# edwindn/rl-agent-for-qubit-array-tuning

Measured on NVIDIA B200. Metric: ground_state_pixels_per_s, higher is better.
Workload: dtype f64

## Files before the change

### rl-agent-for-qubit-array-tuning_b200/csrc/qd_api.cu

```cuda
#include <cuda_runtime.h>
#include <stdarg.h>
#include <stdio.h>
#include <string.h>

#include <new>
#include <stdlib.h>

#include <algorithm>
#include <chrono>
#include <type_traits>
#include <vector>

#include "qd_kernels.cuh"
#include "qd_tunnel.cuh"
#include "qd_tunnel_noda.cuh"
#include "qd_tunnel_enum.cuh"
#include "qd_normalise.cuh"

static_assert(sizeof(qd_scan) == 480, "qd_scan must be 480 bytes (multiple of 16 for the TMA bulk copy)");
static_assert(sizeof(qd_scan) % 16 == 0, "qd_scan size");

struct qd_ctx {
  int device = 0;
  int sm_count = 0;
// ... 155 lines not shown
int issue(qd_ctx* ctx, void (*fn)(P...), long long grid, int threads, size_t smem, cudaStream_t stream, const A&... args) {
  if (smem) {
    const int rc = configure_kernel(ctx, (const void*)fn, smem);
    if (rc) return rc;
  }
  fn<<<(unsigned)std::min(grid, 0x7fffffffLL), threads, smem, stream>>>(args...);
  QD_CUDA(ctx, cudaGetLastError());
  ctx->launches += 1;
  return QD_OK;
}

int order_after_last_launch(qd_ctx* ctx, cudaStream_t stream) {
  if (ctx->have_last && ctx->last_stream != stream) QD_CUDA(ctx, cudaStreamWaitEvent(stream, ctx->last_launch, 0));
  return QD_OK;
}
int mark_launch(qd_ctx* ctx, cudaStream_t stream) {
  QD_CUDA(ctx, cudaEventRecord(ctx->last_launch, stream));
  ctx->last_stream = stream;
  ctx->have_last = true;
  return QD_OK;
}

struct PixelItems { int warps; long long grid; };
PixelItems plan_pixel_items(const qd_ctx* ctx, qd::KArgs& a, long long max_pix, int warps_per_sm) {
  const long long want_items = (long long)ctx->sm_count * warps_per_sm * 4;
  const long long ppi = std::min<long long>(std::max<long long>(((long long)a.n_scan * max_pix) / want_items, 1), 64);
  a.rows_per_item = (int)ppi;
  a.items_per_scan = (int)((max_pix + ppi - 1) / ppi);
  const long long items = (long long)a.n_scan * a.items_per_scan;
  const int warps = (items < (long long)ctx->sm_count * 4) ? 1 : 4;
  return {warps, (items + warps - 1) / warps};
}

int primary_then_fixup(qd_ctx* ctx, const qd::KArgs& g, const PixelItems& p, kernel_fn primary, const qd::KArgs& pa,
                       kernel_fn fallback, int fallback_slot_bytes, bool fix, cudaStream_t stream) {
  if (primary) {
    const int rc = issue(ctx, primary, p.grid, p.warps * 32, (size_t)pa.slot_bytes * p.warps, stream, pa);
    if (rc) return rc;
  }
  if (!fix) return QD_OK;
  qd::KArgs fa = g;
  fa.slot_bytes = fallback_slot_bytes;
  long long grid = p.grid;
  if (primary) {
    fa.fixup = 1;
    fa.mark_ppi = g.rows_per_item;
    fa.rows_per_item = (g.rows_per_item % 8 == 0) ? 8 : g.rows_per_item;
    fa.items_per_scan = (int)((ctx->up_max_pix + fa.rows_per_item - 1) / fa.rows_per_item);
    grid = ((long long)fa.n_scan * fa.items_per_scan + p.warps - 1) / p.warps;
    grid = std::min<long long>(grid, (long long)ctx->sm_count * 32);
  }
  return issue(ctx, fallback, grid, p.warps * 32, (size_t)fa.slot_bytes * p.warps, stream, fa);
}

int tunnel_ground_state(qd_ctx* ctx, int n_scan, const qd_scan* d_scans, const double* d_points, unsigned flags,
                        cudaStream_t stream) {
  const int N = ctx->L.n_dot;
  const kernel_fn gs = pick_dots<2>(N, [](auto n) { return qd::qd_tunnel_gs_kernel<decltype(n)::value>; });
  if (!gs) return fail(ctx, QD_ERR_UNSUPPORTED, "tunnel path needs 2..8 dots, got %d", N);
  int rc = grow(ctx, &ctx->d_nbar, &ctx->nbar_cap, (size_t)ctx->up_pixels * N * sizeof(double));
  if (rc) return rc;
  qd::KArgs g;
  memset(&g, 0, sizeof(g));
  g.L = ctx->L; g.records = ctx->d_records; g.scans = d_scans; g.points = d_points; g.z_out = nullptr;
  g.n_out = nullptr; g.nbar = ctx->d_nbar; g.n_scan = n_scan; g.n_type = QD_N_NONE; g.flags = flags;
  g.status = ctx->d_status;
  g.topt = 7;
  if (const char* e = getenv("QDSIM_TUNNEL_OPT")) g.topt = atoi(e) & 7;
  const long long max_pix = ctx->up_max_pix;
  const char* mono_e = getenv("QDSIM_TUNNEL_MONO");
  if (mono_e && mono_e[0] == '1') {
    g.slot_bytes = qd::qd_tunnel_slot_bytes(ctx->L);
    const PixelItems p = plan_pixel_items(ctx, g, max_pix, 12);
    return issue(ctx, gs, p.grid, p.warps * 32, (size_t)g.slot_bytes * p.warps, stream, g);
  }
  const kernel_fn kr = pick_dots<2>(N, [](auto n) { return qd::qd_tunnel_relax_kernel<decltype(n)::value>; });
  const kernel_fn ks = pick_dots<2>(N, [](auto n) { return qd::qd_tunnel_select_kernel<decltype(n)::value>; });
  const kernel_fn ke = pick_dots<2>(N, [](auto n) { return qd::qd_tunnel_eigen_kernel<decltype(n)::value>; });
  const char* sel_e = getenv("QDSIM_SELECT");
  const kernel_fn ks2 = (sel_e && sel_e[0] == 'b')
                            ? nullptr
                            : pick_dots<4>(N, [](auto n) { return qd::qd_tunnel_select2_kernel<decltype(n)::value>; });
  const char* eig_e = getenv("QDSIM_EIGEN");
  const bool no_fixup = eig_e && eig_e[0] == 'n';
  const kernel_fn ke2 = (eig_e && eig_e[0] == 'h')
                            ? nullptr
                            : pick_dots<2>(N, [](auto n) { return qd::qd_tunnel_eigen2_kernel<decltype(n)::value>; });
  long long chunk_pix = 8LL << 20;
  if (const char* e = getenv("QDSIM_TUNNEL_CHUNK_PIX")) chunk_pix = atoll(e) > 0 ? atoll(e) : chunk_pix;
  const long long spc = std::min<long long>(std::max<long long>(chunk_pix / max_pix, 1), n_scan);
  rc = grow(ctx, &ctx->d_tfloor, &ctx->tfloor_cap, (size_t)spc * max_pix * 8);
  if (rc) return rc;
  rc = grow(ctx, &ctx->d_tkeys, &ctx->tkeys_cap, (size_t)spc * max_pix * 256);
  if (rc) return rc;
  rc = grow(ctx, &ctx->d_tpot, &ctx->tpot_cap, (size_t)spc * max_pix * 128);
  if (rc) return rc;
  g.tfloor = ctx->d_tfloor;
  g.tpot = ctx->d_tpot;
  g.tkeys = ctx->d_tkeys;
  g.tstride = max_pix;
  for (long long c0 = 0; c0 < n_scan; c0 += spc) {
    g.scans = d_scans + c0;
    g.n_scan = (int)std::min<long long>(spc, n_scan - c0);
    qd::KArgs r = g;
    r.rows_per_item = (int)std::min<long long>(1024, max_pix);
    r.items_per_scan = (int)((max_pix + r.rows_per_item - 1) / r.rows_per_item);
    rc = issue(ctx, kr, (long long)r.n_scan * r.items_per_scan, 128, qd::qd_tunnel_relax_smem_bytes(ctx->L), stream, r);
    if (rc) return rc;
    const PixelItems p = plan_pixel_items(ctx, g, max_pix, 16);
    qd::KArgs sa = g;
    sa.slot_bytes = qd::qd_tunnel_select2_slot_bytes(ctx->L);
    rc = primary_then_fixup(ctx, g, p, ks2, sa, ks, qd::qd_tunnel_select_slot_bytes(ctx->L), true, stream);
    if (rc) return rc;
    qd::KArgs ea = g;
    ea.e2_kappa = 4.0f; ea.e2_qsafe = 4.0f; ea.e2_tol = 2e-10f;
    if (const char* e = getenv("QDSIM_E2_KAPPA")) ea.e2_kappa = (float)atof(e);
    if (const char* e = getenv("QDSIM_E2_QSAFE")) ea.e2_qsafe = (float)atof(e);
    if (const char* e = getenv("QDSIM_E2_TOL")) ea.e2_tol = (float)atof(e);
    ea.slot_bytes = qd::qd_tunnel_eigen2_slot_bytes(ctx->L);
    rc = primary_then_fixup(ctx, g, p, ke2, ea, ke, qd::qd_tunnel_eigen_slot_bytes(ctx->L), !no_fixup, stream);
    if (rc) return rc;
  }
  return QD_OK;
}

int launch(qd_ctx* ctx, int n_scan, const qd_scan* d_scans, int max_ny, const double* d_points, float* d_z, void* d_n,
           int n_type, unsigned flags, cudaStream_t stream, int rows_cap = 0, const qd_scan* h_one = nullptr) {
  int rc = order_after_last_launch(ctx, stream);
  if (rc) return rc;
  const bool fast = use_fast_kernel(ctx->L, flags, d_points != nullptr);
  const kernel_fn fn =
      fast ? pick_dots<1>(ctx->L.n_dot, [](auto n) { return qd::qd_scan_fast_kernel<decltype(n)::value>; })
           : pick_kernel(ctx->L, flags, d_points != nullptr);
  if (!fn) return fail(ctx, QD_ERR_UNSUPPORTED, "no kernel for n_dot=%d algorithm=%d", ctx->L.n_dot, ctx->L.algorithm);
  qd::KArgs a;
  memset(&a, 0, sizeof(a));
  if (ctx->L.algorithm == QD_ALG_TUNNEL) {
    rc = tunnel_ground_state(ctx, n_scan, d_scans, d_points, flags, stream);
    if (rc) return rc;
    a.nbar = ctx->d_nbar;
  }
  a.L = ctx->L;
  a.records = ctx->d_records;
  a.scans = d_scans;
  a.points = d_points;
  a.z_out = d_z;
  a.n_out = (n_type == QD_N_NONE) ? nullptr : d_n;
  a.n_scan = n_scan;
  a.n_type = n_type;
  a.flags = flags;
  a.status = ctx->d_status;
  if (h_one && ctx->L.algorithm != QD_ALG_TUNNEL) { a.use_one = 1; a.one = *h_one; }
  a.slot_bytes = fast ? qd::qd_fast_slot_bytes(ctx->L) : qd::qd_slot_bytes(ctx->L);
  const long long target_items = (long long)ctx->sm_count * (fast ? 16 : 12) * 4;
  long long rows = ((long long)n_scan * max_ny) / target_items;
  if (rows < 1) rows = 1;
  if (rows > max_ny) rows = max_ny;
  if (rows_cap > 0 && rows > rows_cap) rows = rows_cap;
  if (flags & QD_FLAG_CARRY_ROWS) rows = max_ny;
  a.rows_per_item = (int)rows;
  a.items_per_scan = (max_ny + a.rows_per_item - 1) / a.rows_per_item;
  a.col_parts = 1;
  if (!(flags & (QD_FLAG_LATCH | QD_FLAG_NOISE | QD_FLAG_PINK | QD_FLAG_CARRY_ROWS)) && rows == 1 &&
      (long long)n_scan * a.items_per_scan < (long long)ctx->sm_count) {
    const long long chunks_x = (ctx->up_max_pix / std::max(1, max_ny) + 31) / 32;
    long long cp = (long long)ctx->sm_count * 2 / std::max<long long>(1, (long long)n_scan * a.items_per_scan);
    cp = std::min<long long>(std::max<long long>(cp, 1), std::max<long long>(chunks_x, 1));
    a.col_parts = (int)cp;
    a.items_per_scan *= a.col_parts;
  }
  const long long total_items = (long long)n_scan * a.items_per_scan;
  int wpc = (total_items < (long long)ctx->sm_count * 4) ? 1 : (fast ? 1 : QD_CTA_WARPS);
  if (const char* e = getenv("QDSIM_WPC")) { const int v = atoi(e); if (v == 1 || v == 2 || v == 4) wpc = v; }
  rc = issue(ctx, fn, (total_items + wpc - 1) / wpc, wpc * 32, (size_t)a.slot_bytes * wpc, stream, a);
  if (rc) return rc;
  return mark_launch(ctx, stream);
}

int check_scan(qd_ctx* ctx, int i, const qd_scan& s) {
  if (s.env_id < 0 || s.env_id >= ctx->n_env)
    return fail(ctx, QD_ERR_INVALID, "scan %d: env_id %d out of range [0,%d)", i, s.env_id, ctx->n_env);
  if (s.nx <= 0 || s.ny <= 0) return fail(ctx, QD_ERR_INVALID, "scan %d: nx, ny must be positive", i);
  if (s.pix_offset < 0) return fail(ctx, QD_ERR_INVALID, "scan %d: negative pix_offset", i);
  return QD_OK;
}

int stage_scans(qd_ctx* ctx, int n_scan, const qd_scan* scans, cudaStream_t stream, int* max_ny,
                bool caller_syncs = false) {
  if (n_scan <= 0) return fail(ctx, QD_ERR_INVALID, "n_scan must be positive");
  if (!scans) return fail(ctx, QD_ERR_INVALID, "scans is NULL");
  const size_t bytes = (size_t)n_scan * sizeof(qd_scan);
  int rc = grow(ctx, &ctx->d_scans, &ctx->scans_cap, bytes);
  if (rc) return rc;
  rc = order_after_last_launch(ctx, stream);
  if (rc) return rc;
  bool pinned = false;
  if (bytes > 64 * 1024) {
    cudaPointerAttributes attr;
    pinned = cudaPointerGetAttributes(&attr, scans) == cudaSuccess && attr.type == cudaMemoryTypeHost;
    if (!pinned) cudaGetLastError();
  }
  const qd_scan* src = scans;
  if (!pinned) {
    if (ctx->staged_pending) {
      QD_CUDA(ctx, cudaEventSynchronize(ctx->staged));
      ctx->staged_pending = false;
    }
    if (ctx->h_scans_cap < bytes) {
      if (ctx->h_scans) cudaFreeHost(ctx->h_scans);
      ctx->h_scans = nullptr;
      ctx->h_scans_cap = 0;
      const size_t want = bytes + bytes / 4 + 4096;
      QD_CUDA(ctx, cudaMallocHost((void**)&ctx->h_scans, want));
      ctx->h_scans_cap = want;
    }
    memcpy(ctx->h_scans, scans, bytes);
    src = ctx->h_scans;
  }
  QD_CUDA(ctx, cudaMemcpyAsync(ctx->d_scans, src, bytes, cudaMemcpyHostToDevice, stream));
  if (!pinned && !caller_syncs) {
    QD_CUDA(ctx, cudaEventRecord(ctx->staged, stream));
    ctx->staged_pending = true;
  }
  ctx->up_n_scan = 0;
  int mny = 0;
  long long ext = 0, mpix = 0;
  for (int i = 0; i < n_scan; ++i) {
    const qd_scan& s = scans[i];
    const long long np_ = (long long)s.nx * s.ny;
    if (s.pix_offset + np_ > ext) ext = s.pix_offset + np_;
    if (np_ > mpix) mpix = np_;
    rc = check_scan(ctx, i, s);
    if (rc) return rc;
    if (s.ny > mny) mny = s.ny;
  }
  *max_ny = mny;
  ctx->up_n_scan = n_scan;
  ctx->up_max_ny = mny;
  ctx->up_pixels = ext;
  ctx->up_max_pix = mpix;
  return QD_OK;
}

int check_status(qd_ctx* ctx) {
  const unsigned st = *reinterpret_cast<volatile unsigned*>(ctx->h_status);
  if (!st) return QD_OK;
  *ctx->h_status = 0u;
  if (st & QD_STATUS_OCC_OVERFLOW)
    return fail(ctx, QD_ERR_INVALID,
                "a scan window reaches 252 or more carriers on a dot: outside the 0..255 range of the uint8 charge map "
                "and of the packed latching keys");
  return fail(ctx, QD_ERR_INVALID, "kernel status 0x%x", st);
}

struct ChunkPlan {
  int n_chunk = 1;
  std::vector<int> cut;
  std::vector<long long> lo, hi;
  bool tiled = true;
};

ChunkPlan plan_chunks(const qd_ctx* ctx, int n_scan, const qd_scan* scans, int align) {
  ChunkPlan P;
  const long long pixels = ctx->up_pixels;
  int n_chunk = n_scan / 2048;
  int chunk_cap = 16;
  if (const char* e = getenv("QDSIM_PIPE_CHUNKS")) chunk_cap = atoi(e) > 0 ? atoi(e) : chunk_cap;
  if (chunk_cap > 16) chunk_cap = 16;
  if (n_chunk > chunk_cap) n_chunk = chunk_cap;
  if (n_chunk < 1) n_chunk = 1;
  if (align < 1) align = 1;
  long long sum = 0;
  for (int i = 0; i < n_scan; ++i) sum += (long long)scans[i].nx * scans[i].ny;
  P.tiled = sum == pixels;
  P.cut.assign(n_chunk + 1, 0);
  {
    std::vector<double> w(n_chunk, 1.0);
    if (n_chunk >= 6) { w[n_chunk - 3] = 0.5; w[n_chunk - 2] = 0.25; w[n_chunk - 1] = 0.125; }
    double tot = 0.0;
    for (double x : w) tot += x;
    if (n_chunk >= 6 && (double)n_scan * w[n_chunk - 1] / tot < 2048.0) { std::fill(w.begin(), w.end(), 1.0); tot = n_chunk; }
    double acc = 0.0;
    for (int c = 0; c < n_chunk; ++c) {
      acc += w[c];
      int at = (int)((double)n_scan * acc / tot);
      at -= at % align;
      P.cut[c + 1] = std::max(at, P.cut[c]);
    }
    P.cut[n_chunk] = n_scan;
  }
  P.lo.assign(n_chunk, 0);
  P.hi.assign(n_chunk, 0);
  bool ok = true;
  for (int c = 0; c < n_chunk && ok; ++c) {
    long long a = -1, b = 0;
    for (int i = P.cut[c]; i < P.cut[c + 1]; ++i) {
      const long long p0 = scans[i].pix_offset, p1 = p0 + (long long)scans[i].nx * scans[i].ny;
      if (a < 0 || p0 < a) a = p0;
      if (p1 > b) b = p1;
    }
    if (a < 0) ok = false;
    P.lo[c] = a; P.hi[c] = b;
    if (c > 0 && P.lo[c] < P.hi[c - 1]) ok = false;
  }
  if (!ok || n_chunk == 1) {
    P.n_chunk = 1;
    P.cut.assign({0, n_scan});
// ... 520 lines not shown
```

### rl-agent-for-qubit-array-tuning_b200/csrc/qd_kernels.cuh

```cuda
#pragma once
#include <math.h>

#include "qd_device.cuh"
#include "qd_layout.h"

namespace qd {

struct KArgs {
  qd_layout L;
  const double* __restrict__ records;
  const qd_scan* __restrict__ scans;
  const double* __restrict__ points;
  float* __restrict__ z_out;
  void* __restrict__ n_out;
  double* __restrict__ nbar;
  unsigned* status;
  unsigned char* tfloor;
  unsigned long long* tkeys;
  double* tpot;
  long long tstride;
  int topt;
  int fixup;
  int mark_ppi;
  float e2_kappa, e2_qsafe, e2_tol;
  int use_one;
  qd_scan one;
  int n_scan;
  int n_type;
  unsigned flags;
  int rows_per_item;
  int items_per_scan;
  int slot_bytes;
  int col_parts;
};

constexpr int QD_DER_DOUBLES = 48;
constexpr int QD_PC_DOUBLES = 8 * 64 + 8 * 16 + 8 + 8 * 32 + 8 * 24;

constexpr int QD_BF_DOUBLES = 8 + 64 + 8;

__host__ __device__ inline int qd_slot_bytes(const qd_layout& L) {
  int b = L.rec_doubles * 8 + (int)sizeof(qd_scan) + QD_DER_DOUBLES * 8 + 16;
  if (L.algorithm == QD_ALG_DEFAULT || L.algorithm == QD_ALG_THRESHOLDED) b += QD_PC_DOUBLES * 8;
  if (L.algorithm == QD_ALG_BRUTE_FORCE) b += QD_BF_DOUBLES * 8;
  return (b + 127) & ~127;
}

#ifndef QD_MIN_BLOCKS
#define QD_MIN_BLOCKS 3
#endif
#ifndef QD_CTA_WARPS
#define QD_CTA_WARPS 4
#endif
constexpr int QD_PC_WAYS = 8;

template <int N>
__device__ __forceinline__ void matvec_smem(const double* __restrict__ M, const double (&x)[N], double (&y)[N]) {
  if constexpr (N % 2 == 0) {
#pragma unroll
    for (int i = 0; i < N; ++i) {
      double s0 = 0.0, s1 = 0.0;
#pragma unroll
      for (int j = 0; j < N; j += 2) {
        const double2 m = *reinterpret_cast<const double2*>(M + i * N + j);
        s0 = fma(m.x, x[j], s0);
        s1 = fma(m.y, x[j + 1], s1);
      }
      y[i] = s0 + s1;
    }
  } else {
#pragma unroll
    for (int i = 0; i < N; ++i) {
      double s0 = 0.0;
#pragma unroll
      for (int j = 0; j < N; ++j) s0 = fma(M[i * N + j], x[j], s0);
      y[i] = s0;
    }
  }
}
struct ProjCache {
  double* aff;
  const double* gsrc;
  double* lin_s;
  uint32_t* keys;
  uint32_t* meta;
  double* mats;
  double* aug;
  int mat_stride;
};

template <int N>
__device__ __noinline__ int proj_cache_build(const ProjCache& pc, const double* __restrict__ cdd, unsigned S, int lane) {
  constexpr int W = 2 * N;
  double* A = pc.aug;
  for (int e = lane; e < N * W; e += 32) {
    const int r = e / W, c = e - r * W;
    double v;
    if (c < N) v = (((S >> r) & 1u) && ((S >> c) & 1u)) ? cdd[r * N + c] : (r == c ? 1.0 : 0.0);
    else v = (r == c - N) ? 1.0 : 0.0;
    A[e] = v;
  }
  __syncwarp();
  for (int k = 0; k < N; ++k) {
    if (!((S >> k) & 1u)) continue;
    const double inv = 1.0 / A[k * W + k];
    double rowk[(N * W + 31) / 32], fr[(N * W + 31) / 32];
#pragma unroll
    for (int t = 0; t < (N * W + 31) / 32; ++t) {
      const int e = lane + 32 * t;
      if (e < N * W) {
        const int r = e / W, c = e - r * W;
        rowk[t] = A[k * W + c] * inv;
        fr[t] = A[r * W + k];
      }
    }
    __syncwarp();
#pragma unroll
    for (int t = 0; t < (N * W + 31) / 32; ++t) {
      const int e = lane + 32 * t;
      if (e < N * W) {
        const int r = e / W;
        A[e] = (r == k) ? rowk[t] : A[e] - fr[t] * rowk[t];
      }
    }
    __syncwarp();
  }
  const int slot = (int)pc.meta[1];
  double* P = pc.mats + slot * pc.mat_stride;
  for (int e = lane; e < N * N; e += 32) {
    const int i = e / N, j = e - i * N;
    double v = (i == j) ? 1.0 : 0.0;
    if ((S >> j) & 1u) {
      for (int q = 0; q < N; ++q)
        if ((S >> q) & 1u) v -= cdd[i * N + q] * A[q * W + N + j];
    }
    if ((S >> i) & 1u) v = 0.0;
    P[e] = v;
  }
  __syncwarp();
  if (pc.gsrc != nullptr && lane < 24) {
    const int t = lane >> 3, i = lane & 7;
    double acc = 0.0;
    if (i < N) {
      const double* src = pc.gsrc + 8 * t;
      for (int j = 0; j < N; ++j) acc = fma(P[i * N + j], src[j], acc);
    }
    pc.aff[slot * 24 + lane] = acc;
  }
  if (lane == 0) {
    pc.keys[slot] = S;
    pc.meta[1] = (uint32_t)((slot + 1) % QD_PC_WAYS);
    if (pc.meta[0] < QD_PC_WAYS) pc.meta[0] += 1;
  }
  __syncwarp();
  return slot;
}

template <int N, bool AFFINE>
__device__ __forceinline__ void relax_lcp(const double (&g)[N], const double* __restrict__ cdd, const ProjCache& pc,
                                          int lane, double fx, double fy, double (&nc)[N]) {
  unsigned act = 0;
#pragma unroll
  for (int j = 0; j < N; ++j) act |= ((unsigned)__double2hiint(g[j]) >> 31) << j;
  bool need = act != 0;
#pragma unroll
  for (int j = 0; j < N; ++j) nc[j] = g[j];
#pragma unroll 1
  for (int round = 0; round <= N; ++round) {
    unsigned pend = __ballot_sync(0xffffffffu, need);
    if (!pend) break;
    bool changed = false;
    while (pend) {
      const int leader = __ffs(pend) - 1;
      const unsigned S = __shfl_sync(0xffffffffu, act, leader);
      const bool member = need && act == S;
      pend &= ~__ballot_sync(0xffffffffu, member);
      const unsigned hit = __ballot_sync(0xffffffffu, lane < (int)pc.meta[0] && pc.keys[lane & (QD_PC_WAYS - 1)] == S &&
                                                          lane < QD_PC_WAYS);
      const int slot = hit ? __ffs(hit) - 1 : proj_cache_build<N>(pc, cdd, S, lane);
      if (member) {
        const double* __restrict__ P = pc.mats + slot * pc.mat_stride;
        unsigned neu = act;
        double wv[N];
        if constexpr (AFFINE) {
          const double* __restrict__ A = pc.aff + slot * 24;
          if constexpr (N % 2 == 0) {
#pragma unroll
            for (int i = 0; i < N; i += 2) {
              const double2 a0 = *reinterpret_cast<const double2*>(A + i);
              const double2 ax = *reinterpret_cast<const double2*>(A + 8 + i);
              const double2 ay = *reinterpret_cast<const double2*>(A + 16 + i);
              wv[i] = fma(fy, ay.x, fma(fx, ax.x, a0.x));
              wv[i + 1] = fma(fy, ay.y, fma(fx, ax.y, a0.y));
            }
          } else {
#pragma unroll
            for (int i = 0; i < N; ++i) wv[i] = fma(fy, A[16 + i], fma(fx, A[8 + i], A[i]));
          }
        } else {
          matvec_smem<N>(P, g, wv);
        }
#pragma unroll
        for (int i = 0; i < N; ++i) {
          const double sacc = ((act >> i) & 1u) ? 0.0 : wv[i];
          nc[i] = sacc;
          neu |= ((unsigned)__double2hiint(sacc) >> 31) << i;
        }
        changed = neu != act;
        act = neu;
      }
      __syncwarp();
    }
    need = changed;
  }
}

template <int N, bool THERMAL, bool AFFINE>
__device__ __forceinline__ void ground_state_box(const double (&g)[N], const double* __restrict__ rec,
                                                 const qd_layout& L, const ProjCache& pc, int lane, bool thresholded,
                                                 double kT, double fx, double fy, double (&nd)[N]) {
  constexpr int NLO = N < 4 ? N : 4;
  constexpr int NHI = N - NLO;
  constexpr int LOC = 1 << NLO;
  const double* __restrict__ cinv = rec + L.o_cinv;
  const double* __restrict__ Q = rec + L.o_q;

  int sgn = 0;
#pragma unroll
  for (int j = 0; j < N; ++j) sgn |= __double2hiint(g[j]);
  const bool neg = sgn < 0;
  double nc[N];
#pragma unroll
  for (int j = 0; j < N; ++j) nc[j] = g[j];
  if (__any_sync(0xffffffffu, neg)) relax_lcp<N, AFFINE>(g, rec + L.o_cdd, pc, lane, fx, fy, nc);

  double f[N], r[N], lin[N];
#pragma unroll
  for (int j = 0; j < N; ++j) {
    f[j] = floor(nc[j]);
    r[j] = f[j] - g[j];
  }
  matvec_smem<N>(cinv, r, lin);
#pragma unroll
  for (int i = 0; i < N; ++i) lin[i] *= 2.0;
  unsigned fixmask = 0, fixval = 0;
  if (thresholded) {
    const double half_thr = 0.5 * rec[L.o_par + QD_PAR_THRESHOLD];
#pragma unroll
    for (int j = 0; j < N; ++j) {
      const double frac = nc[j] - f[j];
      if (!(fabs(frac - 0.5) < half_thr)) {
        fixmask |= 1u << (N - 1 - j);
        if (floor(nc[j] + 0.5) - f[j] == 1.0) fixval |= 1u << (N - 1 - j);
      }
    }
  }
  const unsigned thr_mask = fixmask, thr_val = fixval;
  {
    const double* __restrict__ spos = rec + L.o_spos;
    const double* __restrict__ sneg = rec + L.o_sneg;
    unsigned zmask = 0, omask = 0;
#pragma unroll
    for (int j = 0; j < N; ++j) {
      const unsigned bit = 1u << (N - 1 - j);
      const double aj = lin[j] + cinv[j * N + j];
      zmask |= (aj + sneg[j] > 1e-9) ? bit : 0u;
      omask |= (aj + spos[j] < -1e-9) ? bit : 0u;
    }
    const unsigned add = (zmask | omask) & ~fixmask;
    fixval |= omask & add;
    fixmask |= add;
  }
  const double INF = __longlong_as_double(0x7ff0000000000000LL);
  double llo[LOC];
  double best = INF;
  int bidx = 0;
  const unsigned freeb = ~fixmask & ((1u << N) - 1u);
  const int kfree = __popc(freeb);
  const int kmax = __reduce_max_sync(0xffffffffu, kfree);
  if (kmax <= 4) {
    double* __restrict__ ls = pc.lin_s + lane;
    unsigned idx = fixval, pos = 0;
    double Lsum = 0.0;
    {
      int nfree = 0;
#pragma unroll
      for (int p = 0; p < N; ++p) {
        const double lp = lin[N - 1 - p];
        ls[p * 32] = lp;
        if ((fixval >> p) & 1u) Lsum += lp;
        if ((freeb >> p) & 1u) { pos |= (unsigned)p << (4 * nfree); ++nfree; }
      }
    }
    best = Lsum + Q[idx];
    bidx = (int)idx;
    const unsigned steps = 1u << kmax, mine = 1u << kfree;
#pragma unroll 1
    for (unsigned c = 1; c < steps; ++c) {
      if (c < mine) {
        const unsigned p = (pos >> (4 * (__ffs(c) - 1))) & 15u;
        idx ^= 1u << p;
        const double lp = ls[p * 32];
        Lsum += ((idx >> p) & 1u) ? lp : -lp;
        const double e = Lsum + Q[idx];
        if (e < best || (e == best && (int)idx < bidx)) { best = e; bidx = (int)idx; }
      }
    }
  } else {
  llo[0] = 0.0;
#pragma unroll
  for (int p = 0; p < NLO; ++p)
#pragma unroll
    for (int b = 0; b < (1 << p); ++b) llo[b + (1 << p)] = llo[b] + lin[N - 1 - p];
#pragma unroll
  for (int b = 0; b < LOC; ++b)
    if (((unsigned)b ^ fixval) & fixmask & (LOC - 1)) llo[b] = INF;

  double best_m = INF;
  int best_h = 0;
// ... 597 lines not shown
              }
            });
            if (integral) {
              if (key != key_free) {
#pragma unroll
                for (int j = 0; j < N; ++j) nd[j] = (double)(int)((unsigned)(key >> (8 * j)) & 0xffu);
              }
            } else {
              const int last = 31 - __clz(vmask);
              if (lane == last) {
#pragma unroll
                for (int j = 0; j < N; ++j) d_carry[j] = nd[j];
              }
              __syncwarp();
            }
          }

          double noise_in = 0.0, noise_out = 0.0;
          if (f_noise) {
            const double wn = par[QD_PAR_WHITE] * (double)rnd.z_white;
            if (f_white_out) noise_out = wn; else noise_in = wn;
            const double tamp = par[QD_PAR_TELE_AMP];
            if (tamp != 0.0) {
              if (!tele_init) {
                tele_state = tele_start(f_carry, seed, iy, par);
                tele_init = true;
              }
              const uint32_t flip0 = ((double)rnd.u_tele < par[QD_PAR_P01]) ? 1u : 0u;
              const uint32_t flip1 = ((double)rnd.u_tele < par[QD_PAR_P10]) ? 1u : 0u;
              uint32_t fn = valid ? ((0u ^ flip0) | ((1u ^ flip1) << 1)) : 2u;
#pragma unroll
              for (int d = 1; d < 32; d <<= 1) {
                const uint32_t other = __shfl_up_sync(0xffffffffu, fn, d);
                if (lane >= d) fn = compose2(fn, other);
              }
              const uint32_t st = (fn >> tele_state) & 1u;
              tele_state = __shfl_sync(0xffffffffu, st, 31);
              noise_in += tamp * (double)st;
            }
          }
          if (f_pink && par[QD_PAR_PINK] != 0.0) {
            if (!pink_init) {
              const Philox4 ws = philox4x32_10(seed, (uint64_t)iy, 3u);
              float s0, s1, s2, s3;
              box_muller(ws.w0, ws.w1, s0, s1);
              box_muller(ws.w2, ws.w3, s2, s3);
              __syncwarp();
              if (lane == 0) { d_pink[0] = (double)s0; d_pink[1] = (double)s1; d_pink[2] = (double)s2; d_pink[3] = (double)s3; }
              __syncwarp();
              pink_init = true;
            }
            const Philox4 wp = philox4x32_10(seed, (uint64_t)pix, 2u);
            float e4[4];
            box_muller(wp.w0, wp.w1, e4[0], e4[1]);
            box_muller(wp.w2, wp.w3, e4[2], e4[3]);
            const int last = 31 - __clz(vmask);
            double psum = 0.0;
            double xs_new[4];
#pragma unroll
            for (int k = 0; k < 4; ++k) {
              const double ak = (k == 0) ? 0.60653065971263342 : (k == 1) ? 0.88249690258459546
                              : (k == 2) ? 0.96923323447634413 : 0.99221793826024351;
              double Bk = sqrt(1.0 - ak * ak) * (double)e4[k];
              double ad = ak, apow = 1.0;
#pragma unroll
              for (int d = 1; d < 32; d <<= 1) {
                const double tb = __hiloint2double(__shfl_up_sync(0xffffffffu, __double2hiint(Bk), d),
                                                   __shfl_up_sync(0xffffffffu, __double2loint(Bk), d));
                if (lane >= d) Bk = fma(ad, tb, Bk);
                if ((lane + 1) & d) apow *= ad;
                ad *= ad;
              }
              if ((lane + 1) & 32) apow *= ad;
              const double xk = fma(apow, d_pink[k], Bk);
              xs_new[k] = shfl_f64(xk, last);
              psum += xk;
            }
            __syncwarp();
            if (lane == 0) {
#pragma unroll
              for (int k = 0; k < 4; ++k) d_pink[k] = xs_new[k];
            }
            __syncwarp();
            noise_in += par[QD_PAR_PINK] * 0.5 * psum;
          }

          double base = 0.0;
#pragma unroll
          for (int j = 0; j < N; ++j) base = fma(rec[L.o_sw + j], nd[j] - g[j], base);
          base *= 2.0;
          const double t = (rint(us) + noise_in) - us;
          const double xs = 2.0 * css * inv_gamma;
          const double x0 = fma(css, fma(2.0, t, 1.0), base) * inv_gamma;
          double z;
          if constexpr (ALG == QD_ALG_TUNNEL) {
            double zs = 0.0;
#pragma unroll
            for (int k = -5; k < 5; ++k) {
              const double xk = fma((double)k, xs, x0);
              zs += 1.0 / fma(xk, xk, 1.0);
            }
            z = zs + noise_out;
          } else {
            z = (double)sensor_lorentz10(x0, xs) + noise_out;
          }
          if (f_radial && sc->rad_mode == 1) z = fma((double)rnd.z_rad, (double)radial_amp(sc, (double)ixc, (double)iy), z);
          zf = (float)z;
        } else {
          zf = rnd.z_rad;
#pragma unroll
          for (int j = 0; j < N; ++j) nd[j] = 0.0;
        }

        if (valid) {
          const long long o = pix0 + (long long)iy * nx + ix;
          if (a.z_out) a.z_out[o] = zf;
          if (a.n_type == QD_N_U8) {
            unsigned char* p = reinterpret_cast<unsigned char*>(a.n_out) + o * N;
            if constexpr (N == 8) {
              uint64_t k = 0;
#pragma unroll
              for (int j = 0; j < N; ++j) k |= (uint64_t)(unsigned char)min(255, (int)nd[j]) << (8 * j);
              *reinterpret_cast<uint64_t*>(p) = k;
            } else if constexpr (N == 4) {
              uint32_t k = 0;
#pragma unroll
              for (int j = 0; j < N; ++j) k |= (uint32_t)(unsigned char)min(255, (int)nd[j]) << (8 * j);
              *reinterpret_cast<uint32_t*>(p) = k;
            } else if constexpr (N == 2) {
              const uint16_t k = (uint16_t)((unsigned char)min(255, (int)nd[0]) | ((unsigned char)min(255, (int)nd[1]) << 8));
              *reinterpret_cast<uint16_t*>(p) = k;
            } else {
#pragma unroll
              for (int j = 0; j < N; ++j) p[j] = (unsigned char)min(255, (int)nd[j]);
            }
          } else if (a.n_type == QD_N_F32) {
            float* p = reinterpret_cast<float*>(a.n_out) + o * N;
#pragma unroll
            for (int j = 0; j < N; ++j) p[j] = (float)nd[j];
          } else if (a.n_type == QD_N_F64) {
            double* p = reinterpret_cast<double*>(a.n_out) + o * N;
#pragma unroll
            for (int j = 0; j < N; ++j) p[j] = nd[j];
          }
        }
      }
    }
    __syncwarp();
  }
}


#ifndef QD_FAST_MIN_BLOCKS
#define QD_FAST_MIN_BLOCKS 4
#endif
constexpr int QD_FAST_DER = 32;
constexpr int QD_FAST_PC = 64 + 8 * 16 + 8 + 8 * 32 + QD_PC_WAYS * 24;

__host__ __device__ inline int qd_fast_slot_bytes(const qd_layout& L) {
  const int b = L.rec_doubles * 8 + (int)sizeof(qd_scan) + (QD_FAST_DER + 32 + QD_FAST_PC) * 8 + 16;
  return (b + 127) & ~127;
}

template <int N>
__global__ void __launch_bounds__(QD_CTA_WARPS * 32, QD_FAST_MIN_BLOCKS) qd_scan_fast_kernel(const KArgs a) {
  extern __shared__ __align__(128) unsigned char qd_smem[];
  const int lane = threadIdx.x & 31;
  const int warp = threadIdx.x >> 5;
  const int warps_per_cta = blockDim.x >> 5;
  const qd_layout& L = a.L;

  unsigned char* slot = qd_smem + (size_t)warp * a.slot_bytes;
  double* rec = reinterpret_cast<double*>(slot);
  qd_scan* sc = reinterpret_cast<qd_scan*>(slot + (size_t)L.rec_doubles * 8);
  double* der = reinterpret_cast<double*>(slot + (size_t)L.rec_doubles * 8 + sizeof(qd_scan));
  double* d_g0 = der;
  double* d_gx = der + 8;
  double* d_gy = der + 16;
  double* d_us = der + 24;
  double* d_sg = der + 27;
  double* swt = der + QD_FAST_DER;
  ProjCache pc;
  pc.mats = swt + 32;
  pc.aug = pc.mats + 64;
  pc.keys = reinterpret_cast<uint32_t*>(pc.aug + 8 * 16);
  pc.meta = pc.keys + QD_PC_WAYS;
  pc.lin_s = pc.aug + 8 * 16 + 8;
  pc.aff = pc.lin_s + 8 * 32;
  pc.gsrc = der;
  pc.mat_stride = 0;
  uint64_t* bar = reinterpret_cast<uint64_t*>(pc.aff + QD_PC_WAYS * 24);

  if (lane == 0) mbar_init(bar, 1);
  __syncwarp();
  uint32_t phase = 0;

  const bool f_latch = a.flags & QD_FLAG_LATCH;
  const bool f_noise = a.flags & QD_FLAG_NOISE;
  const bool f_radial = a.flags & QD_FLAG_RADIAL;
  const bool f_carry = a.flags & QD_FLAG_CARRY_ROWS;
  const bool f_white_out = a.flags & QD_FLAG_WHITE_ON_OUTPUT;
  const bool thresholded = L.algorithm == QD_ALG_THRESHOLDED;
  const uint32_t rec_bytes = (uint32_t)L.rec_doubles * 8u;
  const double* __restrict__ cinv = rec + L.o_cinv;
  const double* __restrict__ Q = rec + L.o_q;
  const double* __restrict__ spos = rec + L.o_spos;
  const double* __restrict__ sneg = rec + L.o_sneg;
  const double* __restrict__ sw = rec + L.o_sw;
  const double* par = rec + L.o_par;

  const long long total_items = (long long)a.n_scan * a.items_per_scan;
  for (long long item = (long long)blockIdx.x * warps_per_cta + warp; item < total_items;
       item += (long long)gridDim.x * warps_per_cta) {
    const int scan_id = (int)(item / a.items_per_scan);
    const int part = (int)(item - (long long)scan_id * a.items_per_scan);
    const qd_scan* gscan = a.scans + scan_id;

    stage_item(a, gscan, rec_bytes, rec, sc, bar, phase, lane, a.use_one);
    if (lane == 0) { pc.meta[0] = 0u; pc.meta[1] = 0u; }

    const int nx = sc->nx, ny = sc->ny;
    const ItemWindow w = item_window(a, part, nx, ny);
    if (w.empty) { __syncwarp(); continue; }
    const int row0 = w.row0, row1 = w.row1, cx0 = w.cx0, cx1 = w.cx1;

    item_affine_forms<N>(a, rec, sc, der, lane);
    {
      double t = 0.0;
      const int h = lane & 15;
#pragma unroll
      for (int q = 0; q < 4; ++q) {
        const int p = (lane < 16) ? q : q + 4;
        if (p < N && ((h >> q) & 1)) t += sw[N - 1 - p];
      }
      swt[lane] = t;
    }
    __syncwarp();
    if (lane < 3) {
      double t = 0.0;
      for (int j = 0; j < N; ++j) t = fma(sw[j], der[8 * lane + j], t);
      d_sg[lane] = t;
    }
    __syncwarp();

    const bool latch_on = f_latch && par[QD_PAR_LATCH] != 0.0;
    const bool replace = f_radial && sc->rad_mode == 2;
    const uint64_t seed = sc->seed;
    const long long pix0 = sc->pix_offset;
    const double inv_gamma = 1.0 / sc->peak_width;
    const double css = rec[L.o_css];
    const bool need_rng = f_noise || latch_on || (f_radial && sc->rad_mode != 0);

    uint64_t held_key = 0;
    double held_sn = 0.0;
    bool have_held = false;
    uint32_t tele_state = 0;
    bool tele_init = false;

    for (int iy = row0; iy < row1; ++iy) {
      if (!f_carry) { have_held = false; tele_init = false; }
      for (int c0 = cx0; c0 < cx1; c0 += 32) {
        const int ix = c0 + lane;
        const bool valid = ix < nx;
        const int ixc = valid ? ix : nx - 1;
        const long long pix = (long long)iy * nx + ixc;
        const unsigned vmask = __ballot_sync(0xffffffffu, valid);
        const double fx = (double)ixc, fy = (double)iy;
        const PixelDraws rnd = pixel_draws(need_rng, seed, pix);

        uint64_t key = 0;
        float zf;
        if (!replace) {
          double sn;
          {
            double g[N], nc[N];
            int sgn = 0;
#pragma unroll
            for (int j = 0; j < N; ++j) {
              g[j] = fma(fy, d_gy[j], fma(fx, d_gx[j], d_g0[j]));
              nc[j] = g[j];
              sgn |= __double2hiint(g[j]);
            }
            if (__any_sync(0xffffffffu, sgn < 0)) relax_lcp<N, true>(g, rec + L.o_cdd, pc, lane, fx, fy, nc);
            double r[N], lin[N];
            unsigned fixmask = 0, fixval = 0;
            uint32_t klo = 0, khi = 0;
            sn = 0.0;
#pragma unroll
            for (int j = 0; j < N; ++j) {
              const double fj = floor(nc[j]);
              r[j] = fj - g[j];
              sn = fma(sw[j], fj, sn);
              const uint32_t fi = (uint32_t)__double2int_rz(fj) & 0xffu;
              if (j < 4) klo |= fi << (8 * j); else khi |= fi << (8 * (j - 4));
              if (thresholded) {
                const double frac = nc[j] - fj;
                if (!(fabs(frac - 0.5) < 0.5 * par[QD_PAR_THRESHOLD])) {
                  fixmask |= 1u << (N - 1 - j);
                  if (floor(nc[j] + 0.5) - fj == 1.0) fixval |= 1u << (N - 1 - j);
                }
              }
            }
            key = ((uint64_t)khi << 32) | klo;
            matvec_smem<N>(cinv, r, lin);
            double* __restrict__ ls = pc.lin_s + lane;
            unsigned zmask = 0, omask = 0;
#pragma unroll
            for (int j = 0; j < N; ++j) {
              const unsigned bit = 1u << (N - 1 - j);
              const double l2 = lin[j] + lin[j];
              ls[(N - 1 - j) * 32] = l2;
              const double aj = l2 + cinv[j * N + j];
              zmask |= (aj + sneg[j] > 1e-9) ? bit : 0u;
              omask |= (aj + spos[j] < -1e-9) ? bit : 0u;
            }
            const unsigned add = (zmask | omask) & ~fixmask;
            fixval |= omask & add;
            fixmask |= add;
            const unsigned freeb = ~fixmask & ((1u << N) - 1u);
            const int kfree = __popc(freeb);
            const int kmax = __reduce_max_sync(0xffffffffu, kfree);
            unsigned idx = fixval;
            double Lsum = 0.0;
#pragma unroll
            for (int p = 0; p < N; ++p)
              if ((fixval >> p) & 1u) Lsum += ls[p * 32];
            double best = Lsum + Q[idx];
            unsigned bidx = idx;
            if (kmax > 0) {
              unsigned pos = 0;
              {
                int nfree = 0;
#pragma unroll
                for (int p = 0; p < N; ++p)
                  if ((freeb >> p) & 1u) { pos |= (unsigned)p << (4 * nfree); ++nfree; }
              }
              const unsigned steps = 1u << kmax, mine = 1u << kfree;
#pragma unroll 1
              for (unsigned c = 1; c < steps; ++c) {
                if (c < mine) {
                  const unsigned p = (pos >> (4 * (__ffs(c) - 1))) & 15u;
                  idx ^= 1u << p;
                  const double lp = ls[p * 32];
                  Lsum += ((idx >> p) & 1u) ? lp : -lp;
                  const double e = Lsum + Q[idx];
                  if (e < best || (e == best && idx < bidx)) { best = e; bidx = idx; }
                }
              }
            }
            key += ((((uint64_t)(bidx << (8 - N))) * 0x8040201008040201ULL) & 0x8080808080808080ULL) >> 7;
            sn += swt[bidx & 15u] + swt[16 + (bidx >> 4)];
          }

          if (latch_on) {
            unsigned todo = vmask;
            if (!have_held) {
              held_key = shfl_u64(key, 0);
              held_sn = shfl_f64(sn, 0);
              todo &= ~1u;
              have_held = true;
            }
            latch_chunk(key, held_key, todo, rnd.u_latch, rec, L, lane, [&](int, unsigned rejected, int acl) {
              if ((rejected >> lane) & 1u) sn = held_sn;
              if (acl < 32) held_sn = shfl_f64(sn, acl);
            });
          }

          double noise_in = 0.0, noise_out = 0.0;
          if (f_noise) {
            const double wn = par[QD_PAR_WHITE] * (double)rnd.z_white;
            if (f_white_out) noise_out = wn; else noise_in = wn;
            const double tamp = par[QD_PAR_TELE_AMP];
            if (tamp != 0.0) {
              if (!tele_init) {
                tele_state = tele_start(f_carry, seed, iy, par);
                tele_init = true;
              }
              const unsigned f0 = __ballot_sync(0xffffffffu, valid && (double)rnd.u_tele < par[QD_PAR_P01]);
              const unsigned f1 = __ballot_sync(0xffffffffu, valid && (double)rnd.u_tele < par[QD_PAR_P10]);
              unsigned st_mask = 0u, rem = 0xffffffffu, cur = tele_state;
              while (true) {
                const unsigned m = (cur ? f1 : f0) & rem;
                if (!m) { if (cur) st_mask |= rem; break; }
                const int t = __ffs(m) - 1;
                if (cur) st_mask |= rem & ((1u << t) - 1u);
                cur ^= 1u;
                if (cur) st_mask |= 1u << t;
                rem &= ~((2u << t) - 1u);
                if (!rem) break;
              }
              tele_state = cur;
              noise_in += tamp * (double)((st_mask >> lane) & 1u);
            }
          }

          const double us = fma(fy, d_us[2], fma(fx, d_us[1], d_us[0]));
          const double sg = fma(fy, d_sg[2], fma(fx, d_sg[1], d_sg[0]));
          const double base = 2.0 * (sn - sg);
          const double t = (rint(us) + noise_in) - us;
          const double xs = 2.0 * css * inv_gamma;
          const double x0 = fma(css, fma(2.0, t, 1.0), base) * inv_gamma;
          double z = (double)sensor_lorentz10(x0, xs) + noise_out;
          if (f_radial && sc->rad_mode == 1) z = fma((double)rnd.z_rad, (double)radial_amp(sc, fx, fy), z);
          zf = (float)z;
        } else {
          zf = rnd.z_rad;
        }

        if (valid) {
          const long long o = pix0 + (long long)iy * nx + ix;
          if (a.z_out) a.z_out[o] = zf;
          if (a.n_type == QD_N_U8) {
            unsigned char* p = reinterpret_cast<unsigned char*>(a.n_out) + o * N;
            if constexpr (N == 8) *reinterpret_cast<uint64_t*>(p) = key;
            else if constexpr (N == 4) *reinterpret_cast<uint32_t*>(p) = (uint32_t)key;
            else if constexpr (N == 2) *reinterpret_cast<uint16_t*>(p) = (uint16_t)key;
            else {
#pragma unroll
              for (int j = 0; j < N; ++j) p[j] = (unsigned char)(key >> (8 * j));
            }
          } else if (a.n_type == QD_N_F32) {
            float* p = reinterpret_cast<float*>(a.n_out) + o * N;
#pragma unroll
            for (int j = 0; j < N; ++j) p[j] = (float)(unsigned)((key >> (8 * j)) & 0xffu);
          } else if (a.n_type == QD_N_F64) {
            double* p = reinterpret_cast<double*>(a.n_out) + o * N;
#pragma unroll
            for (int j = 0; j < N; ++j) p[j] = (double)(unsigned)((key >> (8 * j)) & 0xffu);
          }
        }
      }
    }
    __syncwarp();
  }
}

__global__ void qd_build_q_kernel(qd_layout L, double* __restrict__ records, int n_env) {
  const int n = L.n_dot;
  const int per = 1 << n;
  const long long total = (long long)n_env * per;
  for (long long t = (long long)blockIdx.x * blockDim.x + threadIdx.x; t < total; t += (long long)gridDim.x * blockDim.x) {
    const int env = (int)(t / per);
    const unsigned idx = (unsigned)(t - (long long)env * per);
    double* rec = records + (size_t)env * L.rec_doubles;
    const double* cinv = rec + L.o_cinv;
    double s = 0.0;
    for (int i = 0; i < n; ++i) {
      if (!((idx >> (n - 1 - i)) & 1u)) continue;
      for (int j = 0; j < n; ++j)
        if ((idx >> (n - 1 - j)) & 1u) s += cinv[i * n + j];
    }
    rec[L.o_q + idx] = s;
  }
}

template <typename T>
__global__ void __launch_bounds__(256) qd_fma_peak_kernel(T* out, int iters, T a, T b) {
  T x0 = (T)threadIdx.x, x1 = x0 + 1, x2 = x0 + 2, x3 = x0 + 3, x4 = x0 + 4, x5 = x0 + 5, x6 = x0 + 6, x7 = x0 + 7;
  for (int i = 0; i < iters; ++i) {
#pragma unroll
    for (int u = 0; u < 8; ++u) {
      x0 = x0 * a + b; x1 = x1 * a + b; x2 = x2 * a + b; x3 = x3 * a + b;
      x4 = x4 * a + b; x5 = x5 * a + b; x6 = x6 * a + b; x7 = x7 * a + b;
    }
  }
  out[(size_t)blockIdx.x * blockDim.x + threadIdx.x] = x0 + x1 + x2 + x3 + x4 + x5 + x6 + x7;
}

}
```

Baseline: 15.57 billion.

## Raise fast-kernel occupancy by shrinking smem slot and reducing register pressure

Raises the fast kernel's minimum resident blocks per SM from 4 to 5 and derives the work-item target from that. It shrinks the per-warp shared-memory slot by aliasing the projection-cache matrices and augmented storage onto the lin_s scratch area. Register pressure is cut by keeping the inverse peak width, the seed and the pixel offset in shared memory or re-reading them instead of holding them in registers. Per-pixel threshold constants are precomputed into shared memory, and the RNG draw is moved after the ground-state search. The aliasing is safe only if the cache and the enumeration scratch are never live at the same time, and the tighter launch bound may cause register spills.

```diff
diff --git a/rl-agent-for-qubit-array-tuning_b200/csrc/qd_api.cu b/rl-agent-for-qubit-array-tuning_b200/csrc/qd_api.cu
--- a/rl-agent-for-qubit-array-tuning_b200/csrc/qd_api.cu
+++ b/rl-agent-for-qubit-array-tuning_b200/csrc/qd_api.cu
@@ -331,7 +331,7 @@
   a.status = ctx->d_status;
   if (h_one && ctx->L.algorithm != QD_ALG_TUNNEL) { a.use_one = 1; a.one = *h_one; }
   a.slot_bytes = fast ? qd::qd_fast_slot_bytes(ctx->L) : qd::qd_slot_bytes(ctx->L);
-  const long long target_items = (long long)ctx->sm_count * (fast ? 16 : 12) * 4;
+  const long long target_items = (long long)ctx->sm_count * (fast ? qd::QD_FAST_WARPS_PER_SM : 12) * 4;
   long long rows = ((long long)n_scan * max_ny) / target_items;
   if (rows < 1) rows = 1;
   if (rows > max_ny) rows = max_ny;
diff --git a/rl-agent-for-qubit-array-tuning_b200/csrc/qd_kernels.cuh b/rl-agent-for-qubit-array-tuning_b200/csrc/qd_kernels.cuh
--- a/rl-agent-for-qubit-array-tuning_b200/csrc/qd_kernels.cuh
+++ b/rl-agent-for-qubit-array-tuning_b200/csrc/qd_kernels.cuh
@@ -163,8 +163,6 @@
 #pragma unroll
   for (int j = 0; j < N; ++j) act |= ((unsigned)__double2hiint(g[j]) >> 31) << j;
   bool need = act != 0;
-#pragma unroll
-  for (int j = 0; j < N; ++j) nc[j] = g[j];
 #pragma unroll 1
   for (int round = 0; round <= N; ++round) {
     unsigned pend = __ballot_sync(0xffffffffu, need);
@@ -1068,10 +1066,11 @@
 
 
 #ifndef QD_FAST_MIN_BLOCKS
-#define QD_FAST_MIN_BLOCKS 4
+#define QD_FAST_MIN_BLOCKS 5
 #endif
-constexpr int QD_FAST_DER = 32;
-constexpr int QD_FAST_PC = 64 + 8 * 16 + 8 + 8 * 32 + QD_PC_WAYS * 24;
+constexpr int QD_FAST_WARPS_PER_SM = QD_CTA_WARPS * QD_FAST_MIN_BLOCKS;
+constexpr int QD_FAST_DER = 48;
+constexpr int QD_FAST_PC = 8 * 32 + 8 + QD_PC_WAYS * 24;
 
 __host__ __device__ inline int qd_fast_slot_bytes(const qd_layout& L) {
   const int b = L.rec_doubles * 8 + (int)sizeof(qd_scan) + (QD_FAST_DER + 32 + QD_FAST_PC) * 8 + 16;
@@ -1095,14 +1094,16 @@
   double* d_gy = der + 16;
   double* d_us = der + 24;
   double* d_sg = der + 27;
+  double* d_ig = der + 30;
+  double* d_th = der + 32;
   double* swt = der + QD_FAST_DER;
   ProjCache pc;
-  pc.mats = swt + 32;
-  pc.aug = pc.mats + 64;
-  pc.keys = reinterpret_cast<uint32_t*>(pc.aug + 8 * 16);
+  pc.lin_s = swt + 32;
+  pc.mats = pc.lin_s;
+  pc.aug = pc.lin_s + 64;
+  pc.keys = reinterpret_cast<uint32_t*>(pc.lin_s + 8 * 32);
   pc.meta = pc.keys + QD_PC_WAYS;
-  pc.lin_s = pc.aug + 8 * 16 + 8;
-  pc.aff = pc.lin_s + 8 * 32;
+  pc.aff = pc.lin_s + 8 * 32 + 8;
   pc.gsrc = der;
   pc.mat_stride = 0;
   uint64_t* bar = reinterpret_cast<uint64_t*>(pc.aff + QD_PC_WAYS * 24);
@@ -1151,6 +1152,11 @@
       }
       swt[lane] = t;
     }
+    if (lane < N) {
+      const double c = cinv[lane * N + lane];
+      d_th[2 * lane] = (1e-9 - c - sneg[lane]) / 2;
+      d_th[2 * lane + 1] = (-1e-9 - c - spos[lane]) / 2;
+    }
     __syncwarp();
     if (lane < 3) {
       double t = 0.0;
@@ -1161,10 +1167,8 @@
 
     const bool latch_on = f_latch && par[QD_PAR_LATCH] != 0.0;
     const bool replace = f_radial && sc->rad_mode == 2;
-    const uint64_t seed = sc->seed;
-    const long long pix0 = sc->pix_offset;
-    const double inv_gamma = 1.0 / sc->peak_width;
-    const double css = rec[L.o_css];
+    if (lane == 0) *d_ig = 1.0 / sc->peak_width;
+    __syncwarp();
     const bool need_rng = f_noise || latch_on || (f_radial && sc->rad_mode != 0);
 
     uint64_t held_key = 0;
@@ -1182,92 +1186,89 @@
         const long long pix = (long long)iy * nx + ixc;
         const unsigned vmask = __ballot_sync(0xffffffffu, valid);
         const double fx = (double)ixc, fy = (double)iy;
-        const PixelDraws rnd = pixel_draws(need_rng, seed, pix);
 
         uint64_t key = 0;
+        double sn;
+        if (!replace) {
+          double g[N], nc[N];
+          int sgn = 0;
+#pragma unroll
+          for (int j = 0; j < N; ++j) {
+            g[j] = fma(fy, d_gy[j], fma(fx, d_gx[j], d_g0[j]));
+            nc[j] = g[j];
+            sgn |= __double2hiint(g[j]);
+          }
+          if (__any_sync(0xffffffffu, sgn < 0)) {
+            __syncwarp();
+            relax_lcp<N, true>(g, rec + L.o_cdd, pc, lane, fx, fy, nc);
+          }
+          double r[N], lin[N];
+          unsigned fixmask = 0, fixval = 0;
+          uint32_t klo = 0, khi = 0;
+          sn = 0.0;
+#pragma unroll
+          for (int j = 0; j < N; ++j) {
+            const double fj = floor(nc[j]);
+            r[j] = fj - g[j];
+            sn = fma(sw[j], fj, sn);
+            const uint32_t fi = (uint32_t)__double2int_rz(fj) & 0xffu;
+            if (j < 4) klo |= fi << (8 * j); else khi |= fi << (8 * (j - 4));
+            if (thresholded) {
+              const double frac = nc[j] - fj;
+              if (!(fabs(frac - 0.5) < 0.5 * par[QD_PAR_THRESHOLD])) {
+                fixmask |= 1u << (N - 1 - j);
+                if (floor(nc[j] + 0.5) - fj == 1.0) fixval |= 1u << (N - 1 - j);
+              }
+            }
+          }
+          key = ((uint64_t)khi << 32) | klo;
+          matvec_smem<N>(cinv, r, lin);
+          unsigned zmask = 0, omask = 0;
+#pragma unroll
+          for (int j = 0; j < N; ++j) {
+            const unsigned bit = 1u << (N - 1 - j);
+            const double2 th = reinterpret_cast<const double2*>(d_th)[j];
+            zmask |= (lin[j] > th.x) ? bit : 0u;
+            omask |= (lin[j] < th.y) ? bit : 0u;
+          }
+          const unsigned add = (zmask | omask) & ~fixmask;
+          fixval |= omask & add;
+          fixmask |= add;
+          const unsigned freeb = ~fixmask & ((1u << N) - 1u);
+          const int kfree = __popc(freeb);
+          const int kmax = __reduce_max_sync(0xffffffffu, kfree);
+          unsigned idx = fixval;
+          double Lsum = 0.0;
+#pragma unroll
+          for (int p = 0; p < N; ++p)
+            if ((fixval >> p) & 1u) Lsum += lin[N - 1 - p] + lin[N - 1 - p];
+          double best = Lsum + Q[idx];
+          unsigned bidx = idx;
+          if (kmax > 0) {
+            double* __restrict__ ls = pc.lin_s + lane;
+#pragma unroll
+            for (int j = 0; j < N; ++j) ls[(N - 1 - j) * 32] = lin[j] + lin[j];
+            unsigned pos = 0;
+            for (unsigned b = freeb, sh = 0; b; b &= b - 1u, sh += 4) pos |= (unsigned)(__ffs(b) - 1) << sh;
+            const unsigned steps = 1u << kmax, mine = 1u << kfree;
+#pragma unroll 1
+            for (unsigned c = 1; c < steps; ++c) {
+              if (c < mine) {
+                const unsigned p = (pos >> (4 * (__ffs(c) - 1))) & 15u;
+                idx ^= 1u << p;
+                const double lp = ls[p * 32];
+                Lsum += ((idx >> p) & 1u) ? lp : -lp;
+                const double e = Lsum + Q[idx];
+                if (e < best || (e == best && idx < bidx)) { best = e; bidx = idx; }
+              }
+            }
+          }
+          key += ((((uint64_t)(bidx << (8 - N))) * 0x8040201008040201ULL) & 0x8080808080808080ULL) >> 7;
+          sn += swt[bidx & 15u] + swt[16 + (bidx >> 4)];
+        }
+        const PixelDraws rnd = pixel_draws(need_rng, sc->seed, pix);
         float zf;
         if (!replace) {
-          double sn;
-          {
-            double g[N], nc[N];
-            int sgn = 0;
-#pragma unroll
-            for (int j = 0; j < N; ++j) {
-              g[j] = fma(fy, d_gy[j], fma(fx, d_gx[j], d_g0[j]));
-              nc[j] = g[j];
-              sgn |= __double2hiint(g[j]);
-            }
-            if (__any_sync(0xffffffffu, sgn < 0)) relax_lcp<N, true>(g, rec + L.o_cdd, pc, lane, fx, fy, nc);
-            double r[N], lin[N];
-            unsigned fixmask = 0, fixval = 0;
-            uint32_t klo = 0, khi = 0;
-            sn = 0.0;
-#pragma unroll
-            for (int j = 0; j < N; ++j) {
-              const double fj = floor(nc[j]);
-              r[j] = fj - g[j];
-              sn = fma(sw[j], fj, sn);
-              const uint32_t fi = (uint32_t)__double2int_rz(fj) & 0xffu;
-              if (j < 4) klo |= fi << (8 * j); else khi |= fi << (8 * (j - 4));
-              if (thresholded) {
-                const double frac = nc[j] - fj;
-                if (!(fabs(frac - 0.5) < 0.5 * par[QD_PAR_THRESHOLD])) {
-                  fixmask |= 1u << (N - 1 - j);
-                  if (floor(nc[j] + 0.5) - fj == 1.0) fixval |= 1u << (N - 1 - j);
-                }
-              }
-            }
-            key = ((uint64_t)khi << 32) | klo;
-            matvec_smem<N>(cinv, r, lin);
-            double* __restrict__ ls = pc.lin_s + lane;
-            unsigned zmask = 0, omask = 0;
-#pragma unroll
-            for (int j = 0; j < N; ++j) {
-              const unsigned bit = 1u << (N - 1 - j);
-              const double l2 = lin[j] + lin[j];
-              ls[(N - 1 - j) * 32] = l2;
-              const double aj = l2 + cinv[j * N + j];
-              zmask |= (aj + sneg[j] > 1e-9) ? bit : 0u;
-              omask |= (aj + spos[j] < -1e-9) ? bit : 0u;
-            }
-            const unsigned add = (zmask | omask) & ~fixmask;
-            fixval |= omask & add;
-            fixmask |= add;
-            const unsigned freeb = ~fixmask & ((1u << N) - 1u);
-            const int kfree = __popc(freeb);
-            const int kmax = __reduce_max_sync(0xffffffffu, kfree);
-            unsigned idx = fixval;
-            double Lsum = 0.0;
-#pragma unroll
-            for (int p = 0; p < N; ++p)
-              if ((fixval >> p) & 1u) Lsum += ls[p * 32];
-            double best = Lsum + Q[idx];
-            unsigned bidx = idx;
-            if (kmax > 0) {
-              unsigned pos = 0;
-              {
-                int nfree = 0;
-#pragma unroll
-                for (int p = 0; p < N; ++p)
-                  if ((freeb >> p) & 1u) { pos |= (unsigned)p << (4 * nfree); ++nfree; }
-              }
-              const unsigned steps = 1u << kmax, mine = 1u << kfree;
-#pragma unroll 1
-              for (unsigned c = 1; c < steps; ++c) {
-                if (c < mine) {
-                  const unsigned p = (pos >> (4 * (__ffs(c) - 1))) & 15u;
-                  idx ^= 1u << p;
-                  const double lp = ls[p * 32];
-                  Lsum += ((idx >> p) & 1u) ? lp : -lp;
-                  const double e = Lsum + Q[idx];
-                  if (e < best || (e == best && idx < bidx)) { best = e; bidx = idx; }
-                }
-              }
-            }
-            key += ((((uint64_t)(bidx << (8 - N))) * 0x8040201008040201ULL) & 0x8080808080808080ULL) >> 7;
-            sn += swt[bidx & 15u] + swt[16 + (bidx >> 4)];
-          }
-
           if (latch_on) {
             unsigned todo = vmask;
             if (!have_held) {
@@ -1289,7 +1290,7 @@
             const double tamp = par[QD_PAR_TELE_AMP];
             if (tamp != 0.0) {
               if (!tele_init) {
-                tele_state = tele_start(f_carry, seed, iy, par);
+                tele_state = tele_start(f_carry, sc->seed, iy, par);
                 tele_init = true;
               }
               const unsigned f0 = __ballot_sync(0xffffffffu, valid && (double)rnd.u_tele < par[QD_PAR_P01]);
@@ -1314,6 +1315,7 @@
           const double sg = fma(fy, d_sg[2], fma(fx, d_sg[1], d_sg[0]));
           const double base = 2.0 * (sn - sg);
           const double t = (rint(us) + noise_in) - us;
+          const double css = rec[L.o_css], inv_gamma = *d_ig;
           const double xs = 2.0 * css * inv_gamma;
           const double x0 = fma(css, fma(2.0, t, 1.0), base) * inv_gamma;
           double z = (double)sensor_lorentz10(x0, xs) + noise_out;
@@ -1324,7 +1326,7 @@
         }
 
         if (valid) {
-          const long long o = pix0 + (long long)iy * nx + ix;
+          const long long o = sc->pix_offset + (long long)iy * nx + ix;
           if (a.z_out) a.z_out[o] = zf;
           if (a.n_type == QD_N_U8) {
             unsigned char* p = reinterpret_cast<unsigned char*>(a.n_out) + o * N;
```

After: 16.21 billion (median of 6 runs). 1.04x the previous value.
